# moabarar/nemar

Measured on AMD Instinct MI355X. Metric: train images/sec (256x256 A/B pairs), higher is better.
Workload: dtype f32

## Files before the change

### nemar_amd/csrc/conv.hip

```cpp
#define NEMAR_CONV_HIP
#include "common.h"
#include "conv_exact.h"
#include "conv_call.h"
#include "conv_route.h"
#include "pack_plan.h"

#ifdef NEMAR_AB
extern int g_split16_ring3;
extern int g_split16_ksplit_cap;
extern int g_narrow_fwd4;
extern int g_wg_xreg;
extern int g_register_vec4;
extern int g_overlap_per_lane;
void nemar_norm_planes_debug(int bits);
#endif

int nemar_narrow_fwd(const float* x, const float* w, const float* bias, float* y, int N, int C, int H, int W, int K, int R,
                     int pad, int border, int act, float slope, float* part, size_t part_floats, hipStream_t st);
int nemar_narrow_wgrad(const float* x, const float* gy, float* gw, int N, int C, int H, int W, int K, int R, int pad,
                       int border, float* part, hipStream_t st);
void nemar_wgrad2_launch(const float* x0, int C0, const float* x1, int C1, const float* gy, float* gw, float* gb, int N,
                         int H, int W, int K, int OH, int OW, int R, int S, int stride, int pad, int pad_mode,
                         int target_blocks, bool vec_ok, int dbg, float* part, hipStream_t st);
void nemar_sum_partials_pair(const float* part_a, long long stride_a, int splits_a, float* dst_a, long long n_a,
                             const float* part_b, long long stride_b, int splits_b, float* dst_b, long long n_b, bool accumulate, hipStream_t st);
void nemar_sum_partials_fold(const float* part, long long stride, int splits, float* gx, long long planes, int H, int W, int pad,
                             const float* addend, hipStream_t st);
void nemar_sum_partials(const float* part, long long stride, int splits, float* dst, long long n, bool accumulate,
                        hipStream_t st);

namespace {

static thread_local int g_last_route = 0;
static thread_local int g_last_gy_planes = 0;
static NEMAR_SWITCH(int, g_config_epoch, 0);

// ... 326 lines not shown
        const int h = (int)(t % H);
        const long long nc = t / H;
        const float* q = gp + nc * (long long)Hp * Wp;
        const int y0 = h + pad, x0 = w + pad;
        const int y1 = (h >= 1 && h <= pad) ? pad - h : -1, y2 = (h <= H - 2 && h >= H - 1 - pad) ? 2 * (H - 1) - h + pad : -1;
        const int x1 = (w >= 1 && w <= pad) ? pad - w : -1, x2 = (w <= W - 2 && w >= W - 1 - pad) ? 2 * (W - 1) - w + pad : -1;
        auto rowsum = [&](int y) {
            const float* r = q + (long long)y * Wp;
            float v = r[x0];
            if (x1 >= 0) v += r[x1];
            if (x2 >= 0) v += r[x2];
            return v;
        };
        float s = rowsum(y0);
        if (y1 >= 0) s += rowsum(y1);
        if (y2 >= 0) s += rowsum(y2);
        gx[idx] = addend ? s + addend[idx] : s;
    }
}
void fold_padded(const float* padded, float* gx, int H, int W, int pad, long long total, const float* addend, hipStream_t st) {
    hipLaunchKernelGGL(reflect_fold_kernel, dim3(nemar_stream_grid(total, 256)), dim3(256), 0, st, padded, gx, H, W, pad, total, addend);
}

__global__ __launch_bounds__(256) void k7_mf_weights_kernel(const float* __restrict__ w, float* __restrict__ wt, int Ks, int Cb, int dgrad) {
    const int total = 32 * Cb * 7;
    for (int i = blockIdx.x * 256 + threadIdx.x; i < total; i += gridDim.x * 256) {
        const int dy = i % 7, cb = (i / 7) % Cb, m = i / (7 * Cb), ks = m >> 3, dx = m & 7;
        float v = 0.f;
        if (ks < Ks && dx < 7)
            v = dgrad ? w[(((size_t)cb * Ks + ks) * 7 + (6 - dy)) * 7 + (6 - dx)] : w[(((size_t)ks * Cb + cb) * 7 + dy) * 7 + dx];
        wt[i] = v;
    }
}
struct K7MfWtArgs {
    const float* w; float* wt;
    int Ks, Cb, dgrad;
    int gx, gy;
};
__device__ __forceinline__ void k7_mf_wt_body(const K7MfWtArgs& a, int bx, int, int gx) {
    const int total = 32 * a.Cb * 7;
    for (int i = bx * 256 + threadIdx.x; i < total; i += gx * 256) {
        const int dy = i % 7, cb = (i / 7) % a.Cb, m = i / (7 * a.Cb), ks = m >> 3, dx = m & 7;
        float v = 0.f;
        if (ks < a.Ks && dx < 7)
            v = a.dgrad ? a.w[(((size_t)cb * a.Ks + ks) * 7 + (6 - dy)) * 7 + (6 - dx)] : a.w[(((size_t)ks * a.Cb + cb) * 7 + dy) * 7 + dx];
        a.wt[i] = v;
// ... 224 lines not shown
        if (!prepacked) nemar_k7_fm_pack(w, 49, (long long)C * 49, 1, C, K, workspace, st);
        if (L.k7_fold == 2) {
            float* padded = wsf + ((nemar_k7_fm_pack_floats(C) + 3) & ~(size_t)3);
            nemar_k7_fm_conv(gy, K, OH, OW, 6, 0, workspace, nullptr, padded, C, N, H + 6, W + 6, ACT_NONE, 0.f, 0, st);
            fold_padded(padded, gx0, H, W, pad, total, nullptr, st);
        } else {
            nemar_k7_fm_conv(gy, K, OH, OW, L.k7_fold ? 6 : 3, 0, workspace, nullptr, gx0, C, N, H, W, ACT_NONE, 0.f, L.k7_fold, st);
        }
        what = "conv2d_bwd_data (7x7, 16-bit pipe)";
        break;
    case DgradPlan::SPLIT16: {
        if (!prepacked) nemar_split16_pack(w, workspace, K, C, R, 1, g_split16_variant, st);
        const Split16Done done = nemar_split16_conv(gy, workspace, nullptr, gx0, N, H, W, C, K, R, R - 1 - pad, OH, OW, H, W,
                                                    refl ? SPLIT16_DGRAD_REFLECT : SPLIT16_ZERO, call.scratch, g_xcd_map, g_split16_variant, g_tl,
                                                    L.want_gy_planes ? call.gy_planes_out : nullptr, call.src_max, call.src_planes,
                                                    call.src_planes_kind, call.addend, call.out_max, st);
        call.gy_planes_written = done.dual_written;
        call.epilogue_fused = done.epilogue_fused;
        what = "conv2d_bwd_data (split-16)";
        break;
    }
    case DgradPlan::S16G:
    case DgradPlan::S16G_FOLD: {
        const bool fold16 = L.sub == DgradPlan::S16G_FOLD;
        S16gProblem& q = L.q;
        q.src0 = gy; q.src1 = nullptr; q.bias = bias ? bias + mskip : nullptr;
        if (fold16) { q.dst0 = wsf + L.padded_off; q.dst1 = nullptr; q.M0 = q.M; }
        else if (mskip) { q.dst0 = gx1; q.dst1 = nullptr; q.M0 = q.M; }
        else { q.dst0 = gx0; q.dst1 = gx1; q.M0 = C0; }
        if (!prepacked) nemar_s16g_pack(q, L.pl, w + (size_t)mskip * R * S, (long long)R * S, (long long)C * R * S, workspace, st);
        nemar_s16g_conv(q, L.pl, workspace, st);
        if (fold16) fold_padded(q.dst0, gx0, H, W, pad, total, call.addend, st);
        if (fold16 && call.addend) call.addend_done = true;
        what = fold16 ? "conv2d_bwd_data (16-bit pipe on the padded domain + fold)" : "conv2d_bwd_data (16-bit pipe, in-kernel split)";
        break;
    }
    case DgradPlan::EXACT: {
    const bool ring = L.ring, fold = L.fold;
    bool folded = false;
    const int Hd = fold ? H + 2 * pad : H, Wd = fold ? W + 2 * pad : W;
    const int padd = fold ? 0 : pad;
    float* padded = fold ? wsf + L.padded_off : nullptr;
    int cls = 0;
    for (int ph = 0; ph < stride; ++ph)
        for (int pw = 0; pw < stride; ++pw, ++cls) {
            IgemmParams p;
            dgrad_taps(p.taps, R, S, padd, stride, ph, pw);
            const int OHc = (Hd - ph + stride - 1) / stride, OWc = (Wd - pw + stride - 1) / stride;
            if (OHc <= 0 || OWc <= 0) continue;
            const int Mc = C - mskip;
            p.src0 = gy; p.src1 = nullptr; p.C0 = K; p.C1 = 0; p.Hs = OH; p.Ws = OW;
            p.M = Mc; p.Mpad = igemm_mpad(Mc); p.Kred = p.taps.n * K;
            p.bias = bias ? bias + mskip : nullptr;
            if (fold) { p.dst0 = padded; p.dst1 = nullptr; p.M0 = Mc; }
            else if (mskip) { p.dst0 = gx1; p.dst1 = nullptr; p.M0 = Mc; }
// ... 196 lines not shown
    if (key == 6) { g_min_blocks = value > 0 ? value : 384; return NEMAR_OK; }
    if (key == 14) { g_deterministic = value != 0; return NEMAR_OK; }
    if (key == 8) { g_reflect_aux = value != 0; return NEMAR_OK; }
    if (key == 15) { g_xcd_map = value != 0; return NEMAR_OK; }
    if (key == 20) { g_split16 = value != 0; return NEMAR_OK; }
    if (key == 24) { g_s16g = value != 0; return NEMAR_OK; }
    if (key == 25) { g_s16g_min_mmac = value < 0 ? 0 : value; return NEMAR_OK; }
    if (key == 26) { g_s16g_wgrad_first = value != 0; return NEMAR_OK; }
    if (key == 27) { nemar_s16g_tune(0, value); return NEMAR_OK; }
    if (key == 29) { g_s16g_wgrad = value != 0; return NEMAR_OK; }
    if (key == 31) { nemar_norm_planes_debug(value); return NEMAR_OK; }
    if (key == 32) { g_split16_ring3 = value != 0; return NEMAR_OK; }
    if (key == 33) { g_k7 = value != 0; return NEMAR_OK; }
    if (key == 36) { g_split_act = value != 0; return NEMAR_OK; }
    if (key == 43) { g_fold_small = value != 0; return NEMAR_OK; }
    if (key == 37) { g_lds_claim = value; return NEMAR_OK; }
    if (key == 38) { g_wg_xreg = value != 0; return NEMAR_OK; }
    if (key == 39) { g_split16_ksplit_cap = value < 1 ? 1 : (value > 8 ? 8 : value); return NEMAR_OK; }
    if (key == 45) { g_overlap_per_lane = value != 0; return NEMAR_OK; }
    if (key == 44) { g_register_vec4 = value != 0; return NEMAR_OK; }
    if (key == 35) { g_dual_gy = value != 0; return NEMAR_OK; }
    if (key == 34) { nemar_split16_wgrad_tune(value); return NEMAR_OK; }
    if (key == 30) { g_s16g_fold = value != 0; return NEMAR_OK; }
    if (key == 28) { nemar_s16g_tune(1, value); return NEMAR_OK; }
    if (key == 40) { nemar_s16g_tune(2, value); return NEMAR_OK; }
    if (key == 42) { nemar_s16g_tune(4, value); return NEMAR_OK; }
    if (key == 41) { nemar_s16g_tune(3, value); return NEMAR_OK; }
    if (key == 23) { g_split16_min_mmac = value < 0 ? 0 : value; return NEMAR_OK; }
    if (key == 21) { g_split16_variant = value == 3 ? 3 : 4; return NEMAR_OK; }
    if (key == 16) { g_adir = value != 0; return NEMAR_OK; }
    if (key == 17) { g_mt8 = value; return NEMAR_OK; }
    if (key == 19) { g_narrow_fwd4 = value != 0; return NEMAR_OK; }
    if (key == 18) { g_ring = (value == 4 || value == 5) ? value : 3; return NEMAR_OK; }
    if (key == 12) { g_ksplit = value != 0; return NEMAR_OK; }
    if (key == 11) { g_nl4_scalar = value != 0; return NEMAR_OK; }
    if (key == 10) { g_deep64 = value != 0; return NEMAR_OK; }
    if (key == 7) { g_ws2_mt = (value == 1 || value == 2 || value == 4) ? value : 0; return NEMAR_OK; }
    if (key == 5) { g_wgrad_blocks = value > 0 ? value : 512; return NEMAR_OK; }
    nemar_set_error("nemar_tune: unknown key %d", key);
    return NEMAR_EINVAL;
}
#endif

static DgradPlan usual_dgrad(int N, int C, int H, int W, int K, int R, int S, int stride, int pad, int pad_mode) {
    DgradPlan P{};
    if (N <= 0 || C <= 0 || H <= 0 || W <= 0 || K <= 0 || R <= 0 || S <= 0 || stride < 1) return P;
// ... 152 lines not shown
```

### nemar_amd/csrc/conv_route.h

```cpp
#pragma once
#ifndef NEMAR_CONV_HIP
#error "conv_route.h holds conv.hip's own switches: include it from conv.hip only"
#endif
#include "common.h"
#include "conv_exact.h"
#include "conv_split16.h"
#include "conv_s16g.h"
#include "conv_k7.h"

bool nemar_narrow_eligible(int K, int C1, int R, int S, int stride, int N, int OH, int OW);
int nemar_narrow_wgrad_splits(int N, int C, int OH, int OW);
bool nemar_wgrad2_eligible(int K, int OH, int OW, bool gy_aligned16);
void nemar_wgrad2_plan(int K, int J, int P, int target_blocks, int* splits_out, int* pix_per_split_out);

using namespace nemar_exact;

namespace {

static NEMAR_SWITCH(int, g_split16, 1);
static NEMAR_SWITCH(long long, g_split16_min_mmac, 2000);
static NEMAR_SWITCH(int, g_split16_variant, 4);
static NEMAR_SWITCH(int, g_k7, 1);
static NEMAR_SWITCH(int, g_s16g, 1);
static NEMAR_SWITCH(long long, g_s16g_min_mmac, 30);
static NEMAR_SWITCH(int, g_s16g_wgrad, 1);
static NEMAR_SWITCH(int, g_s16g_wgrad_first, 0);
static NEMAR_SWITCH(int, g_s16g_fold, 1);
static NEMAR_SWITCH(int, g_split_act, 1);
static NEMAR_SWITCH(int, g_fold_small, 1);
static NEMAR_SWITCH(int, g_dual_gy, 1);
static NEMAR_SWITCH(int, g_reflect_aux, 1);
static NEMAR_SWITCH(int, g_deterministic, 1);
static NEMAR_SWITCH(int, g_ksplit, 1);
static NEMAR_SWITCH(int, g_narrow, 1);
static NEMAR_SWITCH(int, g_wgrad, 0);
static NEMAR_SWITCH(int, g_wgrad_blocks, 512);

enum { ROUTE_EXACT = 0, ROUTE_NARROW = 1, ROUTE_SPLIT16 = 2, ROUTE_S16G = 3, ROUTE_K7 = 4 };

struct ConvShape {
    int N, C0, C1, H, W, K, R, S, stride, pad, pad_mode;
    int oh = 0, ow = 0;
    int C() const { return C0 + C1; }
    int OH() const { return oh ? oh : (H + 2 * pad - R) / stride + 1; }
    int OW() const { return ow ? ow : (W + 2 * pad - S) / stride + 1; }
    bool refl() const { return pad_mode == BORDER_REFLECT && pad > 0; }
    long long macs() const { return (long long)N * OH() * OW() * K * C() * R * S; }
};
struct ConvFacts {
    bool bias = false;
// ... 174 lines not shown
    const int mode = s.pad_mode == BORDER_REFLECT ? SPLIT16_REFLECT : SPLIT16_ZERO;
    P.sub = FwdPlan::PLAIN;
    if (s.C1 == 0 && P.k7.ok) { P.route = ROUTE_K7; P.sub = FwdPlan::K7_MANY_FEW; }
    else if (g_k7 && s.C1 == 0 && f.act != ACT_TANH && k7_fm) { P.route = ROUTE_K7; P.sub = FwdPlan::K7_FEW_MANY; }
    else if (nemar_narrow_eligible(K, s.C1, R, S, stride, N, OH, OW) && g_narrow) P.route = ROUTE_NARROW;
    else if (g_split16 && s.C1 == 0 && f.act == ACT_NONE && split16_worth_it(N, OH, OW, K, C, R, S) &&
             nemar_split16_eligible(N, H, W, K, C, R, S, stride, pad, mode, g_split16_variant) &&
             f.scratch_bytes && f.scratch_bytes >= nemar_split16_scratch_total(N, H, W, K, C, OH, OW)) P.route = ROUTE_SPLIT16;
    else if (s16g_fwd_problem(P.q, P.pl, N, s.C0, s.C1, H, W, K, R, S, stride, pad, s.pad_mode, f.act, f.slope)) P.route = ROUTE_S16G;
    else {
        const bool split_act = g_split_act && (f.act == ACT_RELU || f.act == ACT_LRELU);
        P.route = ROUTE_EXACT;
        if (P.ksplit > 1 && (f.act == ACT_NONE || split_act)) P.sub = split_act ? FwdPlan::SPLIT_ACT : FwdPlan::SPLIT;
    }
    return P;
}

struct DgradPlan {
    int route;
    enum Sub { K7_MANY_FEW, K7_FEW_MANY, SPLIT16, S16G, S16G_FOLD, EXACT } sub;
    size_t pack_stride, padded_off, w2_off, ring_off, ring_slab_off, slab_off, aux_rows_off, aux_cols_off, total;
    int ring_len, ksplit, ring_ksplit;
    bool ring, fold, fold16, fold_small;
    int k7_fold;
    bool want_gy_planes;
    size_t gy_planes_need;
    int split16_ksplit;
    int mskip;
    bool narrow;
    bool split;
    bool aux_rows;
    K7MfPlan k7;
    S16gProblem q; S16gPlan pl;
};
DgradPlan plan_dgrad(const ConvShape& s, const ConvFacts& f) {
    DgradPlan L;
    const int N = s.N, C = s.C(), H = s.H, W = s.W, K = s.K, R = s.R, S = s.S, stride = s.stride, pad = s.pad, OH = s.OH(), OW = s.OW();
    const bool refl = s.refl();
    L.ring = refl && stride == 1;
    L.fold = refl && !L.ring;
    L.pack_stride = packed_floats(C, K * R * S);
    if (wide_candidates(s).dgrad)
        grow(L.pack_stride, (nemar_split16_pack_bytes(C, K, R) + 3) / 4);
    bool s16g = false;
    L.fold16 = false;
    if (!refl && OH > 0 && OW > 0 && s16g_dgrad_problem(L.q, L.pl, N, C, 0, H, W, K, OH, OW, R, S, stride, pad, ACT_NONE, 0.f)) {
        s16g = true;
        grow(L.pack_stride, ((nemar_s16g_pack_bytes(L.q, L.pl) + 3) / 4 + stride * stride - 1) / (stride * stride));
    } else if (L.ring && g_s16g_fold && R * S <= 9 && OH > 0 && OW > 0 &&
               s16g_dgrad_problem(L.q, L.pl, N, C, 0, H + 2 * pad, W + 2 * pad, K, OH, OW, R, S, 1, 0, ACT_NONE, 0.f)) {
        L.fold16 = true;
        grow(L.pack_stride, (nemar_s16g_pack_bytes(L.q, L.pl) + 3) / 4);
    }
    L.fold_small = L.ring && !L.fold16 && g_fold_small && g_ksplit && C > 4 && (H + 2 * pad) * (W + 2 * pad) <= 1296;
    if (L.fold_small) { L.ring = false; L.fold = true; }
    size_t o = L.pack_stride * (size_t)(stride * stride);
    L.padded_off = o;
    if (L.fold || L.fold16) o += (size_t)N * C * (H + 2 * pad) * (W + 2 * pad);
    L.w2_off = o;
    if (C <= 4) o += (size_t)C * K * R * S;
    L.ring_off = o;
    L.ring_len = L.ring ? 2 * pad * (W + 2 * pad) + 2 * pad * H : 0;
    o += (size_t)N * C * L.ring_len;
    L.ring_ksplit = 1;
    L.ring_slab_off = o;
    if (L.ring) {
        const int tiles = nemar_cdiv(N * L.ring_len, 64) * nemar_cdiv(C, 64), stages = nemar_cdiv(K * R * S, BK);
        int ks = nemar_cdiv(384, tiles);
        if (ks > nemar_cdiv(stages, 8)) ks = nemar_cdiv(stages, 8);
        L.ring_ksplit = normalize_ksplit(K * R * S, ks < 1 ? 1 : ks);
        if (L.ring_ksplit > 1) o += (size_t)L.ring_ksplit * N * C * L.ring_len;
    }
    L.ksplit = 1;
    const int Hs = L.fold_small ? H + 2 * pad : H, Wsl = L.fold_small ? W + 2 * pad : W;
    if (g_ksplit && stride == 1 && (!L.fold || L.fold_small) && C > 4) {
        const int P = N * Hs * Wsl, Kred = K * R * S, stages = nemar_cdiv(Kred, BK);
        if (g_cfg128 == 0 && C > 64 && K % BK == 0) {
            const long long tiles = (long long)nemar_cdiv(C, 128) * nemar_cdiv(P, 128);
            if (tiles < 200 && stages >= 256) {
                int ks = nemar_cdiv(256, (int)tiles);
// ... 140 lines not shown
```

### nemar_amd/csrc/conv_s16g.h

```cpp
#pragma once
#include <hip/hip_runtime.h>
#include <stddef.h>

constexpr int S16G_MAX_TAPS = 64, S16G_MAX_CLS = 4, S16G_CLS_TAPS = 16;

struct S16gProblem {
    const float* src0; const float* src1; int C0, C1;
    int Hs, Ws;
    int N, M, M0;
    float* dst0; float* dst1;
    const float* bias;
    int act; float slope;
    int border;
    int dbg;
    long long* tl;
    int sstride;
    int OHf, OWf, osy, osx;
    int ncls;
    int ntaps[S16G_MAX_CLS], OH[S16G_MAX_CLS], OW[S16G_MAX_CLS], ooy[S16G_MAX_CLS], oox[S16G_MAX_CLS];
    short dy[S16G_MAX_CLS][S16G_MAX_TAPS], dx[S16G_MAX_CLS][S16G_MAX_TAPS];
    int wofs[S16G_MAX_CLS][S16G_MAX_TAPS];
};

struct S16gPlan {
    int ok;
    int MT, NT, ATAPS;
    int TW, RT, tiles_x, tiles_y, mblks, nchunks;
    int HR, HC, HCP, HCH, dymin, dxmin;
    size_t pack_words_per_class;
    int CF;
};
S16gPlan nemar_s16g_plan(const S16gProblem& q);
size_t nemar_s16g_pack_bytes(const S16gProblem& q, const S16gPlan& pl);
void nemar_s16g_pack(const S16gProblem& q, const S16gPlan& pl, const float* w, long long wsm, long long wsc, void* packed,
                     hipStream_t st);
void nemar_s16g_conv(const S16gProblem& q, const S16gPlan& pl, const void* packed, hipStream_t st);

bool nemar_s16g_wgrad_eligible(int N, int C0, int C1, int H, int W, int K, int OH, int OW, int R, int S, int stride, int pad,
                               int pad_mode);
int nemar_s16g_wgrad_slabs(int N, int C0, int C1, int K, int OH, int W, int stride);
int nemar_s16g_wgrad_slabs_max(int N, int C, int K, int OH, int W, int stride);
void nemar_s16g_wgrad(const float* x0, int C0, const float* x1, int C1, const float* gy, float* gw, float* gb, int N, int H, int W,
                      int K, int OH, int OW, int KS, int stride, int pad_mode, float* part, int dbg, hipStream_t st);
void nemar_sum_partials(const float* part, long long stride, int splits, float* dst, long long n, bool accumulate, hipStream_t st);

// ... 7 lines not shown
```

### nemar_amd/csrc/conv_s16g.hip

```cpp
#include "common.h"
#include "conv_s16g.h"
#include "pack_plan.h"

namespace {

typedef float f32x16 __attribute__((ext_vector_type(16)));
typedef _Float16 f16x8 __attribute__((ext_vector_type(8)));
typedef unsigned u32x4 __attribute__((ext_vector_type(4)));

constexpr int BORDER_REFLECT = 1;
constexpr int ACT_RELU = 1, ACT_LRELU = 2, ACT_TANH = 3;
constexpr int BWORDS = 3568;
constexpr int NS4LIM = 2;
typedef float f32x4u __attribute__((ext_vector_type(4), aligned(4)));
constexpr int TEXP = 14;

typedef _Float16 f16x2 __attribute__((ext_vector_type(2)));
__device__ __forceinline__ void split8(const float* v, float s, u32x4& hi, u32x4& lo) {
#pragma unroll
    for (int j = 0; j < 4; ++j) {
        f16x2 h, l;
        h[0] = (_Float16)(v[2 * j] * s);
        h[1] = (_Float16)(v[2 * j + 1] * s);
        l[0] = (_Float16)__builtin_fmaf(v[2 * j], s, -(float)h[0]);
// ... 36 lines not shown
    x = max(x, (unsigned)__builtin_amdgcn_update_dpp(0, (int)x, 0x142, 0xa, 0xf, false));
    x = max(x, (unsigned)__builtin_amdgcn_update_dpp(0, (int)x, 0x143, 0xc, 0xf, false));
    return x;
#endif
}

struct S16gParams {
    const float* src0; const float* src1; int C0, C1, Hs, Ws;
    const u32x4* wp; const unsigned* wmax;
    const float* bias; float* dst0; float* dst1; int M, M0, N;
    int OHf, OWf, osy, osx;
    int border, act; float slope;
    int ncls, xcd;
    int pair;
    long long* tl;
    int dbg;
    int TW, RT, wshift, tiles_x, tiles_y, mblks, nchunks;
    int HR, HC, HCP, HCH, GPR, OFS, hp16, dymin, dxmin;
    int aw16;
    FastDiv fd_gpr;
    long long cls_words;
    int ntaps[S16G_MAX_CLS], OH[S16G_MAX_CLS], OW[S16G_MAX_CLS], ooy[S16G_MAX_CLS], oox[S16G_MAX_CLS];
    int tapoff[S16G_MAX_TAPS];
};

constexpr int ABSMAX_WGS = 64;
__global__ __launch_bounds__(256) void s16g_absmax_kernel(const float* __restrict__ x, long long n, unsigned* out) {
    __shared__ unsigned red[4];
    unsigned m = 0;
    for (long long i = (long long)blockIdx.x * 256 + threadIdx.x; i < n; i += 256ll * ABSMAX_WGS) {
        const unsigned u = __builtin_bit_cast(unsigned, x[i]) & 0x7fffffffu;
        m = max(m, u < 0x7f800000u ? u : 0u);
    }
#pragma unroll
    for (int o = 32; o > 0; o >>= 1) m = max(m, (unsigned)__shfl_xor((int)m, o, 64));
    if ((threadIdx.x & 63) == 0) red[threadIdx.x >> 6] = m;
    __syncthreads();
    if (threadIdx.x == 0) out[blockIdx.x] = max(max(red[0], red[1]), max(red[2], red[3]));
}
__device__ __forceinline__ unsigned absmax_of_partials(const unsigned* part) {
    const u32x4* const q = reinterpret_cast<const u32x4*>(part);
    unsigned m = 0;
#pragma unroll
    for (int i = 0; i < ABSMAX_WGS / 4; ++i) {
        const u32x4 v = q[i];
        m = max(max(m, v[0]), max(max(v[1], v[2]), v[3]));
// ... 389 lines not shown
            for (int ph = 0; ph < 2; ++ph) {
                if (oy >= p.OH[2 * ph] || ox >= p.OW[2 * ph]) continue;
                float* const d0 = dplain + (size_t)(oy * 2 + ph) * p.OWf + (size_t)(ox * 2) + (size_t)(4 * lhi) * plane;
#pragma unroll
                for (int mt = 0; mt < MT; ++mt) {
                    float bv[16];
#pragma unroll
                    for (int r = 0; r < 16; ++r) bv[r] = p.bias ? p.bias[mblk * MB + mt * 32 + (r & 3) + 8 * (r >> 2) + 4 * lhi] : 0.f;
#pragma unroll
                    for (int r = 0; r < 16; ++r) {
                        float o0 = (one_mul ? acc[2 * ph][mt][0][r] * u12 : (acc[2 * ph][mt][0][r] * u1) * u2) + bv[r];
                        float o1 = (one_mul ? acc[2 * ph + 1][mt][0][r] * u12 : (acc[2 * ph + 1][mt][0][r] * u1) * u2) + bv[r];
                        if (p.act == ACT_RELU) { o0 = fmaxf(o0, 0.f); o1 = fmaxf(o1, 0.f); }
                        else if (p.act == ACT_LRELU) { o0 = o0 > 0.f ? o0 : o0 * p.slope; o1 = o1 > 0.f ? o1 : o1 * p.slope; }
                        float* const d = d0 + (size_t)(mt * 32 + (r & 3) + 8 * (r >> 2)) * plane;
                        if (p.pair) *reinterpret_cast<float2*>(d) = make_float2(o0, o1);
                        else { d[0] = o0; d[1] = o1; }
                    }
                    __builtin_amdgcn_sched_barrier(0);
                }
            }
        }
    } else {
#pragma unroll
    for (int mb = 0; mb < NSET; ++mb) {
    const int mbk = CF ? mblk : mblk + mb;
    const int ec = CF ? mb : cls;
    const int OHe = p.OH[ec], OWe = p.OW[ec];
        float bv[MT][16];
    #pragma unroll
        for (int mt = 0; mt < MT; ++mt)
    #pragma unroll
            for (int r = 0; r < 16; ++r) {
                const int m = mbk * MB + mt * 32 + (r & 3) + 8 * (r >> 2) + 4 * lhi;
                bv[mt][r] = p.bias ? p.bias[m < p.M ? m : 0] : 0.f;
            }
        const bool plain = (mbk + 1) * MB <= p.M && ((mbk + 1) * MB <= p.M0 || mbk * MB >= p.M0);
        float* const dplain = mbk * MB >= p.M0 ? p.dst1 + ((size_t)n * M1 + (mbk * MB - p.M0)) * plane : p.dst0 + ((size_t)n * p.M0 + mbk * MB) * plane;
    #pragma unroll
        for (int nt = 0; nt < NT; ++nt) {
            const int oy = oyx[nt] >> 16, ox = oyx[nt] & 0xffff;
            if (oy >= OHe || ox >= OWe) continue;
            const size_t opix = (size_t)(oy * p.osy + p.ooy[ec]) * p.OWf + (size_t)(ox * p.osx + p.oox[ec]);
            if (plain) {
                float* const d0 = dplain + opix + (size_t)(4 * lhi) * plane;
    #define S16G_STORES(EXPR_)                                                                                              \
                _Pragma("unroll") for (int mt = 0; mt < MT; ++mt)                                                           \
                    _Pragma("unroll") for (int r = 0; r < 16; ++r) {                                                        \
                        const float o_ = (one_mul ? acc[mb][mt][nt][r] * u12 : (acc[mb][mt][nt][r] * u1) * u2) + bv[mt][r];         \
                        d0[(size_t)(mt * 32 + (r & 3) + 8 * (r >> 2)) * plane] = (EXPR_);                                   \
                    }
                if (p.act == ACT_RELU) { S16G_STORES(fmaxf(o_, 0.f)) }
                else if (p.act == ACT_LRELU) { S16G_STORES(o_ > 0.f ? o_ : o_ * p.slope) }
                else { S16G_STORES(o_) }
    #undef S16G_STORES
                continue;
            }
    #pragma unroll
            for (int mt = 0; mt < MT; ++mt) {
    #pragma unroll
                for (int r = 0; r < 16; ++r) {
                    const int m = mbk * MB + mt * 32 + (r & 3) + 8 * (r >> 2) + 4 * lhi;
                    if (m >= p.M) continue;
                    float o = (acc[mb][mt][nt][r] * u1) * u2 + bv[mt][r];
                    o = p.act == ACT_RELU ? fmaxf(o, 0.f) : (p.act == ACT_LRELU ? (o > 0.f ? o : o * p.slope) : o);
                    float* const d = m < p.M0 ? p.dst0 + ((size_t)n * p.M0 + m) * plane : p.dst1 + ((size_t)n * M1 + (m - p.M0)) * plane;
                    d[opix] = o;
                }
            }
        }
    }
    }
}

int ilog2(int v) {
    int s = 0;
    while ((1 << s) < v) ++s;
    return s;
}

constexpr int MAX_TIMED = 2048;
hipEvent_t g_tev[MAX_TIMED][2];
int g_tev_made = 0, g_tev_used = 0;
double g_tev_flop = 0.0;
bool g_timing = false;

}

void nemar_s16g_timer(int on) {
    g_timing = on != 0;
    if (on) { g_tev_used = 0; g_tev_flop = 0.0; }
// ... 146 lines not shown
        S16gPackArgs a;
        a.w = w; a.out = (u32x4*)packed; a.M = q.M; a.Cred = C; a.MB = MB; a.mblks = pl.mblks; a.nchunks = pl.nchunks;
        a.wsm = wsm; a.wsc = wsc; a.cls_words = (long long)pl.pack_words_per_class; a.maxbits = mw;
        a.gx = nemar_stream_grid(total, 256); a.gy = q.ncls;
        for (int c = 0; c < S16G_MAX_CLS; ++c) {
            a.ntaps[c] = c < q.ncls ? q.ntaps[c] : 0;
            for (int t = 0; t < S16G_MAX_TAPS; ++t) a.wofs[c][t] = (c < q.ncls && t < q.ntaps[c]) ? q.wofs[c][t] : 0;
        }
        nemar_pack_record_job(PACK_FAM_S16G, &a, a.gx, a.gy);
    }
    S16gProblem qq = q;
    hipLaunchKernelGGL(s16g_pack_kernel, dim3(nemar_stream_grid(total, 256), q.ncls), dim3(256), 0, st, w, (u32x4*)packed, q.M, C, MB,
                       pl.mblks, pl.nchunks, wsm, wsc, (long long)pl.pack_words_per_class, (const unsigned*)mw, qq);
}

void nemar_s16g_conv(const S16gProblem& q, const S16gPlan& pl, const void* packed, hipStream_t st) {
    S16gParams p;
    p.src0 = q.src0; p.src1 = q.src1; p.C0 = q.C0; p.C1 = q.C1; p.Hs = q.Hs; p.Ws = q.Ws;
    p.wp = (const u32x4*)packed;
    p.wmax = pack_max_word(q, pl, const_cast<void*>(packed));
    p.bias = q.bias; p.dst0 = q.dst0; p.dst1 = q.dst1; p.M = q.M; p.M0 = q.M0; p.N = q.N;
    p.OHf = q.OHf; p.OWf = q.OWf; p.osy = q.osy; p.osx = q.osx;
    p.border = q.border; p.act = q.act; p.slope = q.slope; p.dbg = q.dbg; p.tl = q.tl;
    p.TW = pl.TW; p.RT = pl.RT; p.wshift = ilog2(pl.TW); p.tiles_x = pl.tiles_x; p.tiles_y = pl.tiles_y; p.mblks = pl.mblks;
    p.nchunks = pl.nchunks;
    p.HR = pl.HR; p.HC = pl.HC; p.HCP = pl.HCP; p.HCH = pl.HCH; p.hp16 = pl.HR * pl.HCP; p.dymin = pl.dymin; p.dxmin = pl.dxmin;
    p.GPR = pl.HCP / 4;
    p.OFS = pl.dxmin < 0 ? (-pl.dxmin + 3) / 4 * 4 : 0;
    p.fd_gpr = make_fastdiv((unsigned)p.GPR);
    p.cls_words = (long long)pl.pack_words_per_class;
    double flop = 0.0;
    for (int c = 0; c < S16G_MAX_CLS; ++c) {
        const bool on = c < q.ncls;
        p.ntaps[c] = on ? q.ntaps[c] : 0;
        p.OH[c] = on ? q.OH[c] : 0;
        p.OW[c] = on ? q.OW[c] : 0;
        p.ooy[c] = on ? q.ooy[c] : 0;
        p.oox[c] = on ? q.oox[c] : 0;
        if (on) flop += 2.0 * q.N * q.OH[c] * q.OW[c] * (double)q.M * (q.C0 + q.C1) * q.ntaps[c];
    }
    for (int i = 0; i < S16G_MAX_TAPS; ++i) p.tapoff[i] = 0;
    int maxtaps = 0, alltaps = 0;
    for (int c = 0; c < q.ncls; ++c) {
        for (int t = 0; t < q.ntaps[c]; ++t) {
            const int ddy = q.dy[c][t] - pl.dymin, ddx = q.dx[c][t] + p.OFS;
            p.tapoff[pl.CF ? alltaps + t : c * S16G_CLS_TAPS + t] = ddy * pl.HCP + (q.sstride == 2 ? (ddx & 1) * pl.HCH + (ddx >> 1) : ddx);
// ... 76 lines not shown
```

### nemar_amd/csrc/pointwise.hip

```cpp
#include "common.h"
#include "max_words.h"
#include "resize_taps.h"

namespace {

constexpr int ACT_NONE = 0, ACT_RELU = 1, ACT_LRELU = 2, ACT_TANH = 3;

__device__ __forceinline__ float dact_from_out(float y, int act, float slope) {
    if (act == ACT_RELU) return y > 0.f ? 1.f : 0.f;
    if (act == ACT_LRELU) return y > 0.f ? 1.f : slope;
    if (act == ACT_TANH) return 1.f - y * y;
    return 1.f;
}

__global__ __launch_bounds__(256) void act_bwd_kernel(const float* __restrict__ gy, const float* __restrict__ y,
                                                      float* __restrict__ gx, long long n, int act, float slope) {
    const long long n4 = n >> 2;
    const long long stride = (long long)gridDim.x * blockDim.x;
    for (long long i = (long long)blockIdx.x * blockDim.x + threadIdx.x; i < n4; i += stride) {
        const float4 g = reinterpret_cast<const float4*>(gy)[i];
        const float4 o = reinterpret_cast<const float4*>(y)[i];
        float4 r;
        r.x = g.x * dact_from_out(o.x, act, slope);
        r.y = g.y * dact_from_out(o.y, act, slope);
// ... 146 lines not shown
}
__global__ __launch_bounds__(256) void bilinear_up2_bwd_kernel(const float* __restrict__ gy, float* __restrict__ gx, int H,
                                                               int W, long long total_in) {
    const int Wo = 2 * W, Ho = 2 * H;
    for (long long idx = (long long)blockIdx.x * blockDim.x + threadIdx.x; idx < total_in;
         idx += (long long)gridDim.x * blockDim.x) {
        const int w = (int)(idx % W);
        const long long t = idx / W;
        const int h = (int)(t % H);
        const long long nc = t / H;
        int oy[4], ox[4], ny, nx;
        float wy[4], wx[4];
        up2_taps(h, H, oy, wy, ny);
        up2_taps(w, W, ox, wx, nx);
        const float* p = gy + nc * (long long)Ho * Wo;
        float s = 0.f;
        for (int a = 0; a < ny; ++a) {
            float r = 0.f;
            for (int b = 0; b < nx; ++b) r += wx[b] * p[oy[a] * Wo + ox[b]];
            s += wy[a] * r;
        }
        gx[idx] = s;
    }
}

__device__ __forceinline__ void philox4x32_10(unsigned c0, unsigned c1, unsigned c2, unsigned c3, unsigned k0, unsigned k1,
                                              unsigned* out) {
#pragma unroll
    for (int r = 0; r < 10; ++r) {
        const unsigned hi0 = __umulhi(0xD2511F53u, c0), lo0 = 0xD2511F53u * c0;
        const unsigned hi1 = __umulhi(0xCD9E8D57u, c2), lo1 = 0xCD9E8D57u * c2;
        const unsigned n0 = hi1 ^ c1 ^ k0, n1 = lo1, n2 = hi0 ^ c3 ^ k1, n3 = lo0;
        c0 = n0; c1 = n1; c2 = n2; c3 = n3;
        k0 += 0x9E3779B9u;
        k1 += 0xBB67AE85u;
    }
    out[0] = c0; out[1] = c1; out[2] = c2; out[3] = c3;
}

__global__ __launch_bounds__(256) void dropout_kernel(const float* __restrict__ x, float* __restrict__ y, long long n,
                                                      unsigned thresh, float scale, unsigned seed_lo, unsigned seed_hi,
                                                      unsigned offset, unsigned* maxw, const unsigned* obase) {
    if (obase) offset += *obase;
    __shared__ unsigned red[4];
    const long long n4 = (n + 3) >> 2;
    const long long q0 = (long long)blockIdx.y * n4;
// ... 33 lines not shown
        }
    }
}

__global__ __launch_bounds__(256) void crop_flip_normalize_kernel(const float* __restrict__ pool, const int* __restrict__ params,
                                                                  float* __restrict__ y, int C, int H, int W, int Hc, int Wc,
                                                                  float scale, long long total) {
    for (long long idx = (long long)blockIdx.x * blockDim.x + threadIdx.x; idx < total;
         idx += (long long)gridDim.x * blockDim.x) {
        const int w = (int)(idx % Wc);
        long long t = idx / Wc;
        const int h = (int)(t % Hc); t /= Hc;
        const int c = (int)(t % C);
        const int b = (int)(t / C);
        const int4 pr = reinterpret_cast<const int4*>(params)[b];
        const int sx = pr.w ? pr.z + Wc - 1 - w : pr.z + w;
        const float v = pool[(((size_t)pr.x * C + c) * H + (pr.y + h)) * W + sx];
        y[idx] = (v * scale - 0.5f) / 0.5f;
    }
}

}

NEMAR_API int nemar_act_bwd(const float* gy, const float* y, float* gx, long long n, int act, float slope, void* stream) {
    NEMAR_CLEAR_HIP_ERROR();
    NEMAR_REQUIRE(gy && y && gx && n > 0, "act_bwd: bad arguments");
    NEMAR_REQUIRE((((uintptr_t)gy | (uintptr_t)y | (uintptr_t)gx) & 15) == 0, "act_bwd: pointers must be 16-byte aligned");
    hipLaunchKernelGGL(act_bwd_kernel, dim3(nemar_stream_grid(n / 4 + 1, 256)), dim3(256), 0, (hipStream_t)stream, gy, y,
                       gx, n, act, slope);
    NEMAR_CHECK_LAUNCH("act_bwd");
    return NEMAR_OK;
}

namespace {
constexpr int CONCAT_MAX = 8;
struct ConcatArgs { const float* src[CONCAT_MAX]; long long end[CONCAT_MAX]; int k; };
template <bool VEC>
__global__ __launch_bounds__(256) void concat_pieces_kernel(ConcatArgs a, float* __restrict__ dst, long long total) {
    const long long units = VEC ? (total >> 2) : total;
    for (long long u = (long long)blockIdx.x * 256 + threadIdx.x; u < units; u += (long long)gridDim.x * 256) {
        const long long idx = VEC ? (u << 2) : u;
        int j = 0;
        long long beg = 0;
#pragma unroll
        for (int i = 0; i < CONCAT_MAX - 1; ++i)
            if (i + 1 < a.k && idx >= a.end[i]) { j = i + 1; beg = a.end[i]; }
// ... 71 lines not shown
    if ((W & 1) == 0 && (((uintptr_t)x) & 7) == 0)
        hipLaunchKernelGGL(maxpool2_fwd_kernel, grid, block, 0, (hipStream_t)stream, x, y, H, W, Ho, Wo, total);
    else
        hipLaunchKernelGGL(maxpool2_fwd_kernel_unaligned, grid, block, 0, (hipStream_t)stream, x, y, H, W, Ho, Wo, total);
    NEMAR_CHECK_LAUNCH("maxpool2_fwd");
    return NEMAR_OK;
}

NEMAR_API int nemar_maxpool2_bwd(const float* x, const float* gy, const float* addend, float* gx, int planes, int H, int W,
                                 void* stream) {
    NEMAR_CLEAR_HIP_ERROR();
    NEMAR_REQUIRE(x && gy && gx && planes > 0 && H >= 2 && W >= 2, "maxpool2_bwd: bad arguments");
    const long long total = (long long)planes * H * W;
    hipLaunchKernelGGL(maxpool2_bwd_kernel, dim3(nemar_stream_grid(total, 256)), dim3(256), 0, (hipStream_t)stream, x, gy,
                       addend, gx, H, W, H / 2, W / 2, total);
    NEMAR_CHECK_LAUNCH("maxpool2_bwd");
    return NEMAR_OK;
}

NEMAR_API int nemar_bilinear_fwd(const float* x, float* y, int planes, int H, int W, int Ho, int Wo, void* stream) {
    NEMAR_CLEAR_HIP_ERROR();
    NEMAR_REQUIRE(x && y && planes > 0 && H > 0 && W > 0 && Ho > 0 && Wo > 0, "bilinear_fwd: bad arguments");
    const long long total = (long long)planes * Ho * Wo;
    hipLaunchKernelGGL(bilinear_fwd_kernel, dim3(nemar_stream_grid(total, 256)), dim3(256), 0, (hipStream_t)stream, x, y, H,
                       W, Ho, Wo, (float)H / (float)Ho, (float)W / (float)Wo, total);
    NEMAR_CHECK_LAUNCH("bilinear_fwd");
    return NEMAR_OK;
}

NEMAR_API int nemar_bilinear_bwd(const float* gy, float* gx, int planes, int H, int W, int Ho, int Wo, void* stream) {
    NEMAR_CLEAR_HIP_ERROR();
    NEMAR_REQUIRE(gy && gx && planes > 0 && H > 0 && W > 0 && Ho > 0 && Wo > 0, "bilinear_bwd: bad arguments");
    hipStream_t st = (hipStream_t)stream;
    if (Ho == 2 * H && Wo == 2 * W) {
        const long long total = (long long)planes * H * W;
        hipLaunchKernelGGL(bilinear_up2_bwd_kernel, dim3(nemar_stream_grid(total, 256)), dim3(256), 0, st, gy, gx, H, W,
                           total);
    } else if (Ho > 0 && Wo > 0 && H % Ho == 0 && W % Wo == 0 && H / Ho >= 2 && W / Wo >= 2) {
        const long long total = (long long)planes * H * W;
        hipLaunchKernelGGL(bilinear_down_bwd_kernel, dim3(nemar_stream_grid(total, 256)), dim3(256), 0, st, gy, gx, H, W, H / Ho,
                           W / Wo, total);
    } else {
        NEMAR_HIP_CALL(hipMemsetAsync(gx, 0, sizeof(float) * (size_t)planes * H * W, st));
        const long long total = (long long)planes * Ho * Wo;
        hipLaunchKernelGGL(bilinear_bwd_kernel, dim3(nemar_stream_grid(total, 256)), dim3(256), 0, st, gy, gx, H, W, Ho, Wo,
                           (float)H / (float)Ho, (float)W / (float)Wo, total);
    }
    NEMAR_CHECK_LAUNCH("bilinear_bwd");
    return NEMAR_OK;
}

const unsigned* g_dropout_base = nullptr;
namespace {
struct Words8 { unsigned w[8]; };
__global__ void store_words_kernel(unsigned* dst, Words8 v, int n) {
    if ((int)threadIdx.x < n) dst[threadIdx.x] = v.w[threadIdx.x];
}
// ... 60 lines not shown
```

Measured before the change: 282.4.

## Fuse reflect-pad fold into s16g dgrad epilogue and vectorize bilinear up2

For 3x3 reflect-padded dgrad on the 16-bit s16g path, the epilogue now writes interior pixels straight into gx and only the one-pixel border ring into a small ring buffer. A light ring-fold kernel then adds the border contributions, replacing the full padded-domain write and fold pass. Separately, bilinear 2x upsample forward and backward get vectorized kernels that each produce four outputs per thread with float4 stores. This cuts memory traffic, but adds epilogue complexity and a second read-modify-write of the border pixels of gx.

```diff
diff --git a/nemar_amd/csrc/conv.hip b/nemar_amd/csrc/conv.hip
--- a/nemar_amd/csrc/conv.hip
+++ b/nemar_amd/csrc/conv.hip
@@ -12,6 +12,7 @@
 extern int g_wg_xreg;
 extern int g_register_vec4;
 extern int g_overlap_per_lane;
+extern int g_up2_vec;
 void nemar_norm_planes_debug(int bits);
 #endif
 
@@ -384,6 +385,48 @@
     hipLaunchKernelGGL(reflect_fold_kernel, dim3(nemar_stream_grid(total, 256)), dim3(256), 0, st, padded, gx, H, W, pad, total, addend);
 }
 
+__global__ __launch_bounds__(256) void reflect_ring_fold_kernel(const float* __restrict__ ring, float* gx, int H, int W, int planes,
+                                                                const float* __restrict__ addend) {
+    const int t = blockIdx.x * 256 + threadIdx.x;
+    const int per_plane = 2 * W + 2 * (H - 2);
+    if (t >= per_plane) return;
+    int h, w;
+    if (t < W) { h = 1; w = t; }
+    else if (t < 2 * W) { h = H - 2; w = t - W; }
+    else {
+        const int u = t - 2 * W, r = u < H - 2 ? u : u - (H - 2);
+        h = r == 0 ? 0 : (r == H - 3 ? H - 1 : r + 1);
+        w = u < H - 2 ? 1 : W - 2;
+    }
+    const bool up = h == 1, down = h == H - 2, left = w == 1, right = w == W - 2;
+    const int rlen = 2 * (W + 2) + 2 * H;
+    for (int pl = blockIdx.y; pl < planes; pl += gridDim.y) {
+        const float* const q = ring + (size_t)pl * rlen;
+        const size_t idx = ((size_t)pl * H + h) * W + w;
+        float s = gx[idx];
+        if (left) s += q[2 * (W + 2) + h];
+        if (right) s += q[2 * (W + 2) + H + h];
+        if (up) {
+            float v = q[w + 1];
+            if (left) v += q[0];
+            if (right) v += q[W + 1];
+            s += v;
+        }
+        if (down) {
+            const float* const b = q + (W + 2);
+            float v = b[w + 1];
+            if (left) v += b[0];
+            if (right) v += b[W + 1];
+            s += v;
+        }
+        gx[idx] = addend ? s + addend[idx] : s;
+    }
+}
+void fold_ring(const float* ring, float* gx, int H, int W, int planes, const float* addend, hipStream_t st) {
+    hipLaunchKernelGGL(reflect_ring_fold_kernel, dim3(nemar_cdiv(2 * W + 2 * (H - 2), 256), planes < 16384 ? planes : 16384), dim3(256), 0, st,
+                       ring, gx, H, W, planes, addend);
+}
+
 __global__ __launch_bounds__(256) void k7_mf_weights_kernel(const float* __restrict__ w, float* __restrict__ wt, int Ks, int Cb, int dgrad) {
     const int total = 32 * Cb * 7;
     for (int i = blockIdx.x * 256 + threadIdx.x; i < total; i += gridDim.x * 256) {
@@ -654,15 +697,19 @@
     }
     case DgradPlan::S16G:
     case DgradPlan::S16G_FOLD: {
-        const bool fold16 = L.sub == DgradPlan::S16G_FOLD;
+        const bool fold16 = L.sub == DgradPlan::S16G_FOLD, ring16 = fold16 && L.ring16;
         S16gProblem& q = L.q;
         q.src0 = gy; q.src1 = nullptr; q.bias = bias ? bias + mskip : nullptr;
-        if (fold16) { q.dst0 = wsf + L.padded_off; q.dst1 = nullptr; q.M0 = q.M; }
+        if (ring16) {
+            q.dst0 = gx0; q.dst1 = nullptr; q.M0 = q.M;
+            q.fold_H = H; q.fold_W = W; q.fold_ring = wsf + L.padded_off; q.fold_addend = call.addend;
+        } else if (fold16) { q.dst0 = wsf + L.padded_off; q.dst1 = nullptr; q.M0 = q.M; }
         else if (mskip) { q.dst0 = gx1; q.dst1 = nullptr; q.M0 = q.M; }
         else { q.dst0 = gx0; q.dst1 = gx1; q.M0 = C0; }
         if (!prepacked) nemar_s16g_pack(q, L.pl, w + (size_t)mskip * R * S, (long long)R * S, (long long)C * R * S, workspace, st);
         nemar_s16g_conv(q, L.pl, workspace, st);
-        if (fold16) fold_padded(q.dst0, gx0, H, W, pad, total, call.addend, st);
+        if (ring16) fold_ring(q.fold_ring, gx0, H, W, N * C, call.addend, st);
+        else if (fold16) fold_padded(q.dst0, gx0, H, W, pad, total, call.addend, st);
         if (fold16 && call.addend) call.addend_done = true;
         what = fold16 ? "conv2d_bwd_data (16-bit pipe on the padded domain + fold)" : "conv2d_bwd_data (16-bit pipe, in-kernel split)";
         break;
@@ -905,6 +952,8 @@
     if (key == 35) { g_dual_gy = value != 0; return NEMAR_OK; }
     if (key == 34) { nemar_split16_wgrad_tune(value); return NEMAR_OK; }
     if (key == 30) { g_s16g_fold = value != 0; return NEMAR_OK; }
+    if (key == 47) { g_up2_vec = value != 0; return NEMAR_OK; }
+    if (key == 46) { g_s16g_ring = value != 0; return NEMAR_OK; }
     if (key == 28) { nemar_s16g_tune(1, value); return NEMAR_OK; }
     if (key == 40) { nemar_s16g_tune(2, value); return NEMAR_OK; }
     if (key == 42) { nemar_s16g_tune(4, value); return NEMAR_OK; }
diff --git a/nemar_amd/csrc/conv_route.h b/nemar_amd/csrc/conv_route.h
--- a/nemar_amd/csrc/conv_route.h
+++ b/nemar_amd/csrc/conv_route.h
@@ -26,6 +26,7 @@
 static NEMAR_SWITCH(int, g_s16g_wgrad, 1);
 static NEMAR_SWITCH(int, g_s16g_wgrad_first, 0);
 static NEMAR_SWITCH(int, g_s16g_fold, 1);
+static NEMAR_SWITCH(int, g_s16g_ring, 1);
 static NEMAR_SWITCH(int, g_split_act, 1);
 static NEMAR_SWITCH(int, g_fold_small, 1);
 static NEMAR_SWITCH(int, g_dual_gy, 1);
@@ -246,6 +247,7 @@
     size_t pack_stride, padded_off, w2_off, ring_off, ring_slab_off, slab_off, aux_rows_off, aux_cols_off, total;
     int ring_len, ksplit, ring_ksplit;
     bool ring, fold, fold16, fold_small;
+    bool ring16;
     int k7_fold;
     bool want_gy_planes;
     size_t gy_planes_need;
@@ -280,6 +282,7 @@
     if (L.fold_small) { L.ring = false; L.fold = true; }
     size_t o = L.pack_stride * (size_t)(stride * stride);
     L.padded_off = o;
+    L.ring16 = L.fold16 && g_s16g_ring && pad == 1 && R == 3 && S == 3 && H >= 4 && W >= 4;
     if (L.fold || L.fold16) o += (size_t)N * C * (H + 2 * pad) * (W + 2 * pad);
     L.w2_off = o;
     if (C <= 4) o += (size_t)C * K * R * S;
diff --git a/nemar_amd/csrc/conv_s16g.h b/nemar_amd/csrc/conv_s16g.h
--- a/nemar_amd/csrc/conv_s16g.h
+++ b/nemar_amd/csrc/conv_s16g.h
@@ -20,7 +20,11 @@
     int ntaps[S16G_MAX_CLS], OH[S16G_MAX_CLS], OW[S16G_MAX_CLS], ooy[S16G_MAX_CLS], oox[S16G_MAX_CLS];
     short dy[S16G_MAX_CLS][S16G_MAX_TAPS], dx[S16G_MAX_CLS][S16G_MAX_TAPS];
     int wofs[S16G_MAX_CLS][S16G_MAX_TAPS];
+    int fold_H = 0, fold_W = 0;
+    float* fold_ring = nullptr;
+    const float* fold_addend = nullptr;
 };
+inline int s16g_ring_len(int H, int W) { return 2 * (W + 2) + 2 * H; }
 
 struct S16gPlan {
     int ok;
diff --git a/nemar_amd/csrc/conv_s16g.hip b/nemar_amd/csrc/conv_s16g.hip
--- a/nemar_amd/csrc/conv_s16g.hip
+++ b/nemar_amd/csrc/conv_s16g.hip
@@ -82,6 +82,9 @@
     long long cls_words;
     int ntaps[S16G_MAX_CLS], OH[S16G_MAX_CLS], OW[S16G_MAX_CLS], ooy[S16G_MAX_CLS], oox[S16G_MAX_CLS];
     int tapoff[S16G_MAX_TAPS];
+    int fold_H, fold_W;
+    float* fold_ring;
+    const float* fold_addend;
 };
 
 constexpr int ABSMAX_WGS = 64;
@@ -517,6 +520,7 @@
             }
         }
     } else {
+    if (__builtin_expect(p.fold_H == 0, 1)) {
 #pragma unroll
     for (int mb = 0; mb < NSET; ++mb) {
     const int mbk = CF ? mblk : mblk + mb;
@@ -562,6 +566,73 @@
                     float* const d = m < p.M0 ? p.dst0 + ((size_t)n * p.M0 + m) * plane : p.dst1 + ((size_t)n * M1 + (m - p.M0)) * plane;
                     d[opix] = o;
                 }
+            }
+        }
+    }
+    return;
+    }
+    if (p.fold_H) {
+        const int FH = p.fold_H, FW = p.fold_W;
+        const size_t hw = (size_t)FH * FW, rl = (size_t)(2 * (FW + 2) + 2 * FH);
+#pragma unroll
+        for (int mb = 0; mb < NSET; ++mb) {
+            const int mbk = mblk + mb;
+            const bool plain = (mbk + 1) * MB <= p.M;
+            const size_t row0 = (size_t)n * p.M + mbk * MB + 4 * lhi;
+#pragma unroll
+            for (int nt = 0; nt < NT; ++nt) {
+                const int oy = oyx[nt] >> 16, ox = oyx[nt] & 0xffff;
+                if (oy >= p.OH[0] || ox >= p.OW[0]) continue;
+                const bool inner = oy >= 1 && oy <= FH && ox >= 1 && ox <= FW;
+                const int iofs = (oy - 1) * FW + (ox - 1);
+                const int rofs = oy == 0 ? ox : oy == FH + 1 ? FW + 2 + ox : ox == 0 ? 2 * (FW + 2) + oy - 1 : 2 * (FW + 2) + FH + oy - 1;
+                const bool fadd = inner && oy != 2 && oy != FH - 1 && ox != 2 && ox != FW - 1;
+    #define S16G_FOLD_VALUE(MT_, R_) ((one_mul ? acc[mb][MT_][nt][R_] * u12 : (acc[mb][MT_][nt][R_] * u1) * u2) + 0.f)
+                if (plain && inner) {
+                    float* const d0 = p.dst0 + row0 * hw + (size_t)iofs;
+                    if (p.fold_addend) {
+                        const float* const a0 = p.fold_addend + row0 * hw + (size_t)iofs;
+    #pragma unroll
+                        for (int mt = 0; mt < MT; ++mt) {
+                            float av[16];
+    #pragma unroll
+                            for (int r = 0; r < 16; ++r) av[r] = fadd ? a0[(size_t)(mt * 32 + (r & 3) + 8 * (r >> 2)) * hw] : 0.f;
+    #pragma unroll
+                            for (int r = 0; r < 16; ++r) {
+                                const float o = S16G_FOLD_VALUE(mt, r);
+                                d0[(size_t)(mt * 32 + (r & 3) + 8 * (r >> 2)) * hw] = fadd ? o + av[r] : o;
+                            }
+                        }
+                    } else {
+    #pragma unroll
+                        for (int mt = 0; mt < MT; ++mt)
+    #pragma unroll
+                            for (int r = 0; r < 16; ++r) d0[(size_t)(mt * 32 + (r & 3) + 8 * (r >> 2)) * hw] = S16G_FOLD_VALUE(mt, r);
+                    }
+                } else if (plain) {
+                    float* const d0 = p.fold_ring + row0 * rl + (size_t)rofs;
+    #pragma unroll
+                    for (int mt = 0; mt < MT; ++mt)
+    #pragma unroll
+                        for (int r = 0; r < 16; ++r) d0[(size_t)(mt * 32 + (r & 3) + 8 * (r >> 2)) * rl] = S16G_FOLD_VALUE(mt, r);
+                } else {
+                    const size_t fplane = inner ? hw : rl;
+                    const size_t fidx = row0 * fplane + (size_t)(inner ? iofs : rofs);
+                    float* const fd = (inner ? p.dst0 : p.fold_ring) + fidx;
+                    const bool radd = fadd && p.fold_addend;
+                    const float* const fa = p.fold_addend + (radd ? fidx : 0);
+    #pragma unroll
+                    for (int mt = 0; mt < MT; ++mt) {
+    #pragma unroll
+                        for (int r = 0; r < 16; ++r) {
+                            const int ml = mt * 32 + (r & 3) + 8 * (r >> 2);
+                            if (mbk * MB + ml + 4 * lhi >= p.M) continue;
+                            const float o = (acc[mb][mt][nt][r] * u1) * u2 + 0.f;
+                            fd[(size_t)ml * fplane] = radd ? o + fa[(size_t)ml * fplane] : o;
+                        }
+                    }
+                }
+    #undef S16G_FOLD_VALUE
             }
         }
     }
@@ -754,6 +825,7 @@
     p.bias = q.bias; p.dst0 = q.dst0; p.dst1 = q.dst1; p.M = q.M; p.M0 = q.M0; p.N = q.N;
     p.OHf = q.OHf; p.OWf = q.OWf; p.osy = q.osy; p.osx = q.osx;
     p.border = q.border; p.act = q.act; p.slope = q.slope; p.dbg = q.dbg; p.tl = q.tl;
+    p.fold_H = q.fold_H; p.fold_W = q.fold_W; p.fold_ring = q.fold_ring; p.fold_addend = q.fold_addend;
     p.TW = pl.TW; p.RT = pl.RT; p.wshift = ilog2(pl.TW); p.tiles_x = pl.tiles_x; p.tiles_y = pl.tiles_y; p.mblks = pl.mblks;
     p.nchunks = pl.nchunks;
     p.HR = pl.HR; p.HC = pl.HC; p.HCP = pl.HCP; p.HCH = pl.HCH; p.hp16 = pl.HR * pl.HCP; p.dymin = pl.dymin; p.dxmin = pl.dxmin;
diff --git a/nemar_amd/csrc/pointwise.hip b/nemar_amd/csrc/pointwise.hip
--- a/nemar_amd/csrc/pointwise.hip
+++ b/nemar_amd/csrc/pointwise.hip
@@ -192,6 +192,118 @@
         }
         gx[idx] = s;
     }
+}
+
+__device__ __forceinline__ float pick4(int k, float c0, float c1, float c2, float c3) {
+    return k == 0 ? c0 : k == 1 ? c1 : k == 2 ? c2 : c3;
+}
+__global__ __launch_bounds__(256) void bilinear_up2_fwd_vec_kernel(const float* __restrict__ x, float* __restrict__ y, int H, int W,
+                                                                   int planes, int lq) {
+    const int Ho = 2 * H, Wo = 2 * W, Q = W >> 1;
+    const int q = (blockIdx.x << lq) + (threadIdx.x & ((1 << lq) - 1));
+    if (q >= Q) return;
+    const int rb = 256 >> lq;
+    const int base = 2 * q - 1;
+    const int cl = base < 0 ? 0 : base, cr = base + 3 > W - 1 ? W - 1 : base + 3;
+    for (int pl = blockIdx.z; pl < planes; pl += gridDim.z) {
+        const float* const xp = x + (size_t)pl * H * W;
+        float* const yp = y + (size_t)pl * Ho * Wo;
+        for (int j = blockIdx.y * rb + (threadIdx.x >> lq); j <= H; j += gridDim.y * rb) {
+            const bool va = j >= 1, vb = j < H;
+            const Tap1D ta = tap1d(va ? 2 * j - 1 : 2 * j, H, 0.5f), tb = tap1d(vb ? 2 * j : 2 * j - 1, H, 0.5f);
+            const float* const r0 = xp + tb.i0 * W;
+            const float* const r1 = xp + tb.i1 * W;
+            const float2 m0 = *reinterpret_cast<const float2*>(r0 + 2 * q), m1 = *reinterpret_cast<const float2*>(r1 + 2 * q);
+            const float a0 = r0[cl], a3 = r0[cr], b0 = r1[cl], b3 = r1[cr];
+            float oa[4], ob[4];
+#pragma unroll
+            for (int e = 0; e < 4; ++e) {
+                const Tap1D tw = tap1d(4 * q + e, W, 0.5f);
+                const int k0 = tw.i0 - base, k1 = tw.i1 - base;
+                const float c00 = pick4(k0, a0, m0.x, m0.y, a3), c01 = pick4(k1, a0, m0.x, m0.y, a3);
+                const float c10 = pick4(k0, b0, m1.x, m1.y, b3), c11 = pick4(k1, b0, m1.x, m1.y, b3);
+                oa[e] = resize_blend(c00, c01, c10, c11, tw, ta);
+                ob[e] = resize_blend(c00, c01, c10, c11, tw, tb);
+            }
+            if (va) *reinterpret_cast<float4*>(yp + (size_t)(2 * j - 1) * Wo + 4 * q) = make_float4(oa[0], oa[1], oa[2], oa[3]);
+            if (vb) *reinterpret_cast<float4*>(yp + (size_t)(2 * j) * Wo + 4 * q) = make_float4(ob[0], ob[1], ob[2], ob[3]);
+        }
+    }
+}
+
+struct Up2Row { float l, v[8], r; };
+__device__ __forceinline__ Up2Row up2_load_row(const float* __restrict__ g, int q, bool has_l, bool has_r) {
+    Up2Row t;
+    const float4 a = *reinterpret_cast<const float4*>(g + 8 * q), b = *reinterpret_cast<const float4*>(g + 8 * q + 4);
+    t.l = has_l ? g[8 * q - 1] : 0.f;
+    t.r = has_r ? g[8 * q + 8] : 0.f;
+    t.v[0] = a.x; t.v[1] = a.y; t.v[2] = a.z; t.v[3] = a.w; t.v[4] = b.x; t.v[5] = b.y; t.v[6] = b.z; t.v[7] = b.w;
+    return t;
+}
+template <int E>
+__device__ __forceinline__ float up2_row_sum(const Up2Row& t, int w, int W) {
+    float r = 0.f;
+    r += (w == 0 ? 1.f : 0.75f) * t.v[2 * E];
+    r += (w == W - 1 ? 1.f : 0.75f) * t.v[2 * E + 1];
+    if (w + 1 < W) r += 0.25f * (E == 3 ? t.r : t.v[E == 3 ? 0 : 2 * E + 2]);
+    if (w >= 1) r += 0.25f * (E == 0 ? t.l : t.v[E == 0 ? 0 : 2 * E - 1]);
+    return r;
+}
+__global__ __launch_bounds__(256) void bilinear_up2_bwd_vec_kernel(const float* __restrict__ gy, float* __restrict__ gx, int H, int W,
+                                                                   int planes, int lq) {
+    const int Wo = 2 * W, Q = W >> 2;
+    const int q = (blockIdx.x << lq) + (threadIdx.x & ((1 << lq) - 1));
+    if (q >= Q) return;
+    const int rb = 256 >> lq;
+    const bool has_l = q > 0, has_r = 8 * q + 8 < Wo;
+    const int w0 = 4 * q;
+    for (int pl = blockIdx.z; pl < planes; pl += gridDim.z) {
+        const float* const gp = gy + (size_t)pl * (2 * H) * Wo;
+        float* const xp = gx + (size_t)pl * H * W;
+        for (int h = blockIdx.y * rb + (threadIdx.x >> lq); h < H; h += gridDim.y * rb) {
+            const bool up = h >= 1, down = h + 1 < H;
+            const float* const g0 = gp + (size_t)(2 * h) * Wo;
+            const Up2Row t0 = up2_load_row(g0, q, has_l, has_r), t1 = up2_load_row(g0 + Wo, q, has_l, has_r);
+            Up2Row t2 = {}, t3 = {};
+            if (down) t2 = up2_load_row(g0 + 2 * Wo, q, has_l, has_r);
+            if (up) t3 = up2_load_row(g0 - Wo, q, has_l, has_r);
+            const float wy0 = h == 0 ? 1.f : 0.75f, wy1 = h == H - 1 ? 1.f : 0.75f;
+            float o[4];
+#define UP2_TEXEL(E_)                                                             \
+            {                                                                     \
+                float s = 0.f;                                                    \
+                s += wy0 * up2_row_sum<E_>(t0, w0 + E_, W);                       \
+                s += wy1 * up2_row_sum<E_>(t1, w0 + E_, W);                       \
+                if (down) s += 0.25f * up2_row_sum<E_>(t2, w0 + E_, W);           \
+                if (up) s += 0.25f * up2_row_sum<E_>(t3, w0 + E_, W);             \
+                o[E_] = s;                                                        \
+            }
+            UP2_TEXEL(0) UP2_TEXEL(1) UP2_TEXEL(2) UP2_TEXEL(3)
+#undef UP2_TEXEL
+            *reinterpret_cast<float4*>(xp + (size_t)h * W + w0) = make_float4(o[0], o[1], o[2], o[3]);
+        }
+    }
+}
+
+struct Up2Launch { dim3 grid; int lq; };
+Up2Launch up2_launch(int groups, int rows, int planes) {
+    Up2Launch L;
+    L.lq = 0;
+    while ((1 << L.lq) < groups && L.lq < 8) ++L.lq;
+    const int rb = 256 >> L.lq;
+    const int gx = nemar_cdiv(groups, 1 << L.lq);
+    int gy = nemar_cdiv(rows, rb);
+    if (gy > 65535) gy = 65535;
+    long long gz = 8192 / ((long long)gx * gy);
+    if (gz < 1) gz = 1;
+    if (gz > planes) gz = planes;
+    if (gz > 65535) gz = 65535;
+    gz = nemar_cdiv(planes, nemar_cdiv(planes, gz));
+    L.grid = dim3(gx, gy, (unsigned)gz);
+    return L;
+}
+bool up2_vec_ok(const void* a, const void* b, int W) {
+    return (W & 3) == 0 && (((uintptr_t)a | (uintptr_t)b) & 15) == 0;
 }
 
 __device__ __forceinline__ void philox4x32_10(unsigned c0, unsigned c1, unsigned c2, unsigned c3, unsigned k0, unsigned k1,
@@ -271,6 +383,8 @@
 
 }
 
+NEMAR_SWITCH(int, g_up2_vec, 1);
+
 NEMAR_API int nemar_act_bwd(const float* gy, const float* y, float* gx, long long n, int act, float slope, void* stream) {
     NEMAR_CLEAR_HIP_ERROR();
     NEMAR_REQUIRE(gy && y && gx && n > 0, "act_bwd: bad arguments");
@@ -388,8 +502,13 @@
     NEMAR_CLEAR_HIP_ERROR();
     NEMAR_REQUIRE(x && y && planes > 0 && H > 0 && W > 0 && Ho > 0 && Wo > 0, "bilinear_fwd: bad arguments");
     const long long total = (long long)planes * Ho * Wo;
-    hipLaunchKernelGGL(bilinear_fwd_kernel, dim3(nemar_stream_grid(total, 256)), dim3(256), 0, (hipStream_t)stream, x, y, H,
-                       W, Ho, Wo, (float)H / (float)Ho, (float)W / (float)Wo, total);
+    if (g_up2_vec && Ho == 2 * H && Wo == 2 * W && up2_vec_ok(x, y, W)) {
+        const Up2Launch L = up2_launch(W / 2, H + 1, planes);
+        hipLaunchKernelGGL(bilinear_up2_fwd_vec_kernel, L.grid, dim3(256), 0, (hipStream_t)stream, x, y, H, W, planes, L.lq);
+    } else {
+        hipLaunchKernelGGL(bilinear_fwd_kernel, dim3(nemar_stream_grid(total, 256)), dim3(256), 0, (hipStream_t)stream, x, y, H,
+                           W, Ho, Wo, (float)H / (float)Ho, (float)W / (float)Wo, total);
+    }
     NEMAR_CHECK_LAUNCH("bilinear_fwd");
     return NEMAR_OK;
 }
@@ -398,7 +517,10 @@
     NEMAR_CLEAR_HIP_ERROR();
     NEMAR_REQUIRE(gy && gx && planes > 0 && H > 0 && W > 0 && Ho > 0 && Wo > 0, "bilinear_bwd: bad arguments");
     hipStream_t st = (hipStream_t)stream;
-    if (Ho == 2 * H && Wo == 2 * W) {
+    if (g_up2_vec && Ho == 2 * H && Wo == 2 * W && up2_vec_ok(gy, gx, W)) {
+        const Up2Launch L = up2_launch(W / 4, H, planes);
+        hipLaunchKernelGGL(bilinear_up2_bwd_vec_kernel, L.grid, dim3(256), 0, st, gy, gx, H, W, planes, L.lq);
+    } else if (Ho == 2 * H && Wo == 2 * W) {
         const long long total = (long long)planes * H * W;
         hipLaunchKernelGGL(bilinear_up2_bwd_kernel, dim3(nemar_stream_grid(total, 256)), dim3(256), 0, st, gy, gx, H, W,
                            total);
```

Result: no change. 284.0 (median of 6 runs) (+0.6%).
